# douban/tfmesos

Measured on NVIDIA B200. Metric: ps_push_pull_GBps, higher is better.
Workload: dtype f32

## Files before the change

tfmesos_b200/csrc/psx.cu:

```cuda
#include <cuda.h>
#include <cuda_runtime.h>
#include <unistd.h>

#include <atomic>
#include <cstdarg>
#include <cstdio>
#include <cstring>
#include <mutex>
#include <thread>
#include <unordered_map>
#include <vector>

#include "psx.h"
#include "psx_kernels.cuh"

using namespace psx;

namespace {

thread_local char g_err[512] = "";

int fail(int code, const char *fmt, ...)
{
    va_list ap;
// ... 9 lines not shown
        if (e_ != cudaSuccess)                                                         \
            return fail(PSX_ECUDA, "%s failed: %s (%s:%d)", #expr, cudaGetErrorString(e_), \
                        __FILE__, __LINE__);                                           \
    } while (0)

struct DeviceGuard {
    int prev = -1;
    cudaError_t err = cudaSuccess;
    explicit DeviceGuard(int device)
    {
        err = cudaGetDevice(&prev);
        if (err == cudaSuccess && prev != device) err = cudaSetDevice(device);
        else if (err == cudaSuccess) prev = -1;
    }
    ~DeviceGuard()
    {
        if (prev >= 0) cudaSetDevice(prev);
    }
};
#define PSX_DEVICE(dev)                                                                  \
    DeviceGuard guard_(dev);                                                             \
    if (guard_.err != cudaSuccess)                                                       \
        return fail(PSX_ECUDA, "selecting device %d: %s", (int)(dev), cudaGetErrorString(guard_.err))

typedef CUresult (*WaitValue32Fn)(CUstream, CUdeviceptr, cuuint32_t, unsigned int);
WaitValue32Fn g_wait32 = nullptr;
std::once_flag g_wait_once;

int resolve_memops()
{
    std::call_once(g_wait_once, [] {
        void *fn = nullptr;
        cudaDriverEntryPointQueryResult q;
        if (cudaGetDriverEntryPoint("cuStreamWaitValue32", &fn, cudaEnableDefault, &q) ==
                cudaSuccess &&
            q == cudaDriverEntryPointSuccess)
            g_wait32 = (WaitValue32Fn)fn;
    });
    if (!g_wait32) return fail(PSX_ECUDA, "cuStreamWaitValue32 not available from the driver");
    return PSX_OK;
}

int stream_wait_geq(void *stream, unsigned int *flag, uint32_t value)
{
    int rc = resolve_memops();
    if (rc) return rc;
    CUresult r = g_wait32((CUstream)stream, (CUdeviceptr)(uintptr_t)flag, value,
                          CU_STREAM_WAIT_VALUE_GEQ);
    if (r != CUDA_SUCCESS) return fail(PSX_ECUDA, "cuStreamWaitValue32 failed: CUresult %d", (int)r);
    return PSX_OK;
}

constexpr uint32_t kMagic = 0x50535831u;
constexpr size_t kHeaderBytes = 4096;
constexpr uint64_t kPadElems = 1024;

enum Kind : uint32_t { KIND_SHARD = 1, KIND_CLIENT = 2, KIND_BUFFER = 3, KIND_MAILBOX = 4 };

struct HandleBlob {
    uint32_t magic, abi, kind;
    int32_t device;
    uint64_t pid, local_id, nelem, nelem_pad;
    int32_t opt, n_slots, wire;
    uint32_t pad;
    cudaIpcMemHandle_t ipc;
};
static_assert(sizeof(HandleBlob) == PSX_HANDLE_BYTES, "handle blob size");

int state_arrays(int opt)
{
    switch (opt) {
    case PSX_OPT_SGD: return OptTraits<PSX_OPT_SGD>::kState;
    case PSX_OPT_ADAM: return OptTraits<PSX_OPT_ADAM>::kState;
    case PSX_OPT_MOMENTUM: return OptTraits<PSX_OPT_MOMENTUM>::kState;
    case PSX_OPT_ADAGRAD: return OptTraits<PSX_OPT_ADAGRAD>::kState;
    case PSX_OPT_RMSPROP: return OptTraits<PSX_OPT_RMSPROP>::kState;
    default: return -1;
    }
}

struct Layout {
    uint64_t nelem = 0, nelem_pad = 0;
    int opt = 0, n_slots = 0, wire = 0;
    size_t wire_bytes() const { return wire == PSX_BF16 ? 2 : 4; }
    int n_state() const { return state_arrays(opt); }
    size_t off_var() const { return kHeaderBytes; }
    size_t off_m() const { return off_var() + nelem_pad * 4; }
    size_t off_v() const { return off_m() + (n_state() >= 1 ? nelem_pad * 4 : 0); }
    size_t off_slots() const { return off_v() + (n_state() >= 2 ? nelem_pad * 4 : 0); }
    size_t total() const { return off_slots() + (size_t)n_slots * nelem_pad * wire_bytes(); }
};

struct Mapped {
    char *base = nullptr;
    bool ipc = false;
    int device = 0;
};

struct Bound {
    Mapped grad, param;
    uint64_t elem_off = 0;
    bool valid = false;
};

struct Server;
struct Shard {
    int device = 0;
    Server *server = nullptr;
    std::recursive_mutex serve_mu;
    Layout lay;
    char *base = nullptr;
    int sm_count = 148;
    Mapped client_map[PSX_MAX_SLOTS];
    unsigned int *mirror[PSX_MAX_SLOTS] = {};
    Bound bound[PSX_MAX_SLOTS];
    Mapped mailbox_map[PSX_MAX_SLOTS];
    unsigned int *mailbox[PSX_MAX_SLOTS] = {};
    const float *mc_grad = nullptr;
    float *mc_param = nullptr;
    int mc_members = 0;
    ShardHeader *hdr() const { return (ShardHeader *)base; }
    float *var() const { return (float *)(base + lay.off_var()); }
    float *m() const { return (float *)(base + lay.off_m()); }
    float *v() const { return (float *)(base + lay.off_v()); }
    char *slot(int s) const { return base + lay.off_slots() + (size_t)s * lay.nelem_pad * lay.wire_bytes(); }
};

struct Client {
    int device = 0;
    int slot = 0;
    Layout lay;
    Mapped shard;
    ClientBlock *block = nullptr;
    cudaStream_t poll_stream = nullptr;
    int sm_count = 148;
    ShardHeader *hdr() const { return (ShardHeader *)shard.base; }
    float *var() const { return (float *)(shard.base + lay.off_var()); }
    char *my_slot() const { return shard.base + lay.off_slots() + (size_t)slot * lay.nelem_pad * lay.wire_bytes(); }
};

struct Mailbox {
    int device = 0;
    unsigned int *counter = nullptr;
};

struct TensorList {
    uint64_t client_id = 0;
    int device = 0;
    ListChunk *d_chunks = nullptr;
    int n_chunks = 0;
    int sm_count = 148;
};

struct Buffer {
    int device = 0;
    uint64_t nbytes = 0;
    char *base = nullptr;
};

std::mutex g_mu;
std::unordered_map<uint64_t, Shard *> g_shards;
std::unordered_map<uint64_t, Client *> g_clients;
std::unordered_map<uint64_t, Buffer *> g_buffers;
std::unordered_map<uint64_t, TensorList *> g_lists;
std::unordered_map<uint64_t, Mailbox *> g_mailboxes;
std::atomic<uint64_t> g_next_id{1};
std::atomic<uint64_t> g_launches{0};

template <typename T> T *find(std::unordered_map<uint64_t, T *> &m, uint64_t id)
{
    std::lock_guard<std::mutex> lk(g_mu);
    auto it = m.find(id);
    return it == m.end() ? nullptr : it->second;
}

int sm_count_of(int device)
{
    int n = 148;
    cudaDeviceGetAttribute(&n, cudaDevAttrMultiProcessorCount, device);
    return n > 0 ? n : 148;
}

int enable_peer(int device, int peer);

int open_blob(const HandleBlob &b, int device, Mapped *out)
{
    out->device = b.device;
    if (b.pid == (uint64_t)getpid()) {
        int prc = enable_peer(device, b.device);
        if (prc) return prc;
        std::lock_guard<std::mutex> lk(g_mu);
        char *base = nullptr;
        if (b.kind == KIND_SHARD) {
            auto it = g_shards.find(b.local_id);
            if (it != g_shards.end()) base = it->second->base;
        } else if (b.kind == KIND_CLIENT) {
            auto it = g_clients.find(b.local_id);
            if (it != g_clients.end()) base = (char *)it->second->block;
        } else if (b.kind == KIND_BUFFER) {
            auto it = g_buffers.find(b.local_id);
            if (it != g_buffers.end()) base = it->second->base;
        } else if (b.kind == KIND_MAILBOX) {
            auto it = g_mailboxes.find(b.local_id);
            if (it != g_mailboxes.end()) base = (char *)it->second->counter;
        }
        if (!base) return fail(PSX_EINVAL, "handle refers to an object this process no longer has");
        out->base = base;
        out->ipc = false;
        return PSX_OK;
    }
    PSX_DEVICE(device);
    void *p = nullptr;
    CU_TRY(cudaIpcOpenMemHandle(&p, b.ipc, cudaIpcMemLazyEnablePeerAccess));
    out->base = (char *)p;
    out->ipc = true;
    return PSX_OK;
}

void close_mapped(Mapped &m)
{
    if (m.ipc && m.base) cudaIpcCloseMemHandle(m.base);
    m.base = nullptr;
    m.ipc = false;
}

int check_blob(const void *handle, uint32_t kind, HandleBlob *out)
{
    if (!handle) return fail(PSX_EINVAL, "null handle");
    memcpy(out, handle, sizeof(HandleBlob));
    if (out->magic != kMagic) return fail(PSX_EINVAL, "not a psx handle");
    if (out->abi != PSX_ABI_VERSION)
        return fail(PSX_EABI, "handle from ABI %u, library is ABI %d", out->abi, PSX_ABI_VERSION);
    if (out->kind != kind) return fail(PSX_EINVAL, "handle kind %u, expected %u", out->kind, kind);
    return PSX_OK;
}

int enable_peer(int device, int peer)
{
    if (device == peer) return PSX_OK;
    int can = 0;
    CU_TRY(cudaDeviceCanAccessPeer(&can, device, peer));
    if (!can) return fail(PSX_ECUDA, "device %d cannot access peer %d", device, peer);
    PSX_DEVICE(device);
    cudaError_t e = cudaDeviceEnablePeerAccess(peer, 0);
    if (e == cudaErrorPeerAccessAlreadyEnabled) {
        cudaGetLastError();
        return PSX_OK;
    }
    if (e != cudaSuccess) return fail(PSX_ECUDA, "cudaDeviceEnablePeerAccess(%d->%d): %s", device, peer, cudaGetErrorString(e));
    return PSX_OK;
}

inline int grid_for(size_t work_items, int threads, int sm_count, int ctas_per_sm)
{
    size_t need = (work_items + threads - 1) / threads;
    size_t cap = (size_t)sm_count * ctas_per_sm;
    if (need < 1) need = 1;
    return (int)(need < cap ? need : cap);
}

#define LAUNCH_CHECK()                                                              \
    do {                                                                            \
        cudaError_t e_ = cudaGetLastError();                                        \
        if (e_ != cudaSuccess)                                                      \
            return fail(PSX_ECUDA, "kernel launch failed: %s (%s:%d)",              \
                        cudaGetErrorString(e_), __FILE__, __LINE__);                \
        g_launches.fetch_add(1, std::memory_order_relaxed);                         \
    } while (0)

int launch_copy(void *dst, int dst_t, const void *src, int src_t, uint64_t n, int sm_count,
                unsigned int *ticket, unsigned int *flag, uint32_t seq, cudaStream_t st,
                unsigned int *arrivals = nullptr, unsigned int *stamp_word = nullptr,
                uint32_t stamp = 0)
{
    if (n == 0 && flag == nullptr) return PSX_OK;
    const size_t sb = src_t == PSX_BF16 ? 2 : 4, db = dst_t == PSX_BF16 ? 2 : 4;
    const int vec_ok = (((uintptr_t)src % (4 * sb)) == 0) && (((uintptr_t)dst % (4 * db)) == 0);
    const size_t items = vec_ok ? ((n >> 2) + kCopyUnroll - 1) / kCopyUnroll : n;
    const int grid = grid_for(items ? items : 1, kCopyThreads, sm_count, 8);
#define PSX_COPY(S, D)                                                                        \
    k_copy<S, D><<<grid, kCopyThreads, 0, st>>>((D *)dst, (const S *)src, (size_t)n, vec_ok, \
                                                 ticket, flag, arrivals, seq, stamp_word, stamp)
    if (src_t == PSX_F32 && dst_t == PSX_F32) PSX_COPY(float, float);
    else if (src_t == PSX_F32 && dst_t == PSX_BF16) PSX_COPY(float, __nv_bfloat16);
    else if (src_t == PSX_BF16 && dst_t == PSX_F32) PSX_COPY(__nv_bfloat16, float);
    else if (src_t == PSX_BF16 && dst_t == PSX_BF16) PSX_COPY(__nv_bfloat16, __nv_bfloat16);
    else return fail(PSX_EINVAL, "unknown dtype %d/%d", src_t, dst_t);
#undef PSX_COPY
    LAUNCH_CHECK();
    return PSX_OK;
}

struct ApplyRange {
    size_t off, n;
    int finish;
    unsigned int consume = 0;
    int divisor = 0;
};

template <int OPT, int MODE, bool SCATTER, typename SRC>
void launch_apply_t(Shard *s, SRC src, int count, const PeerSet &peers, cudaStream_t st,
                    const ApplyRange &r)
{
    const size_t n4 = r.n / 4;
    const int grid = grid_for(n4 ? n4 : 1, kApplyThreads, s->sm_count, 3);
    k_apply<OPT, MODE, SCATTER, SRC><<<grid, kApplyThreads, 0, st>>>(
        s->hdr(), (float4 *)(s->var() + r.off), (float4 *)(s->m() + r.off),
        (float4 *)(s->v() + r.off), src, count, n4, peers, r.finish, r.consume,
        r.divisor ? r.divisor : count);
}

template <bool SCATTER, typename SRC>
int launch_apply(Shard *s, int mode, SRC src, int count, const PeerSet &peers, cudaStream_t st,
                 ApplyRange r = ApplyRange{0, 0, 1, 0, 0})
{
    if (r.n == 0 && r.off == 0) r.n = s->lay.nelem_pad;
#define PSX_AP(O, M) launch_apply_t<O, M, SCATTER, SRC>(s, src, count, peers, st, r)
#define PSX_AP3(O)                                                                            \
    if (mode == PSX_MODE_ASYNC_ORDERED) PSX_AP(O, PSX_MODE_ASYNC_ORDERED);                    \
    else if (mode == PSX_MODE_SUM) PSX_AP(O, PSX_MODE_SUM);                                   \
    else if (mode == PSX_MODE_SYNC_MEAN) PSX_AP(O, PSX_MODE_SYNC_MEAN);                       \
    else return fail(PSX_EINVAL, "unknown optimizer/mode %d/%d", opt, mode)
    const int opt = s->lay.opt;
    if (opt == PSX_OPT_SGD) { PSX_AP3(PSX_OPT_SGD); }
    else if (opt == PSX_OPT_ADAM) { PSX_AP3(PSX_OPT_ADAM); }
    else if (opt == PSX_OPT_MOMENTUM) { PSX_AP3(PSX_OPT_MOMENTUM); }
    else if (opt == PSX_OPT_ADAGRAD) { PSX_AP3(PSX_OPT_ADAGRAD); }
    else if (opt == PSX_OPT_RMSPROP) { PSX_AP3(PSX_OPT_RMSPROP); }
    else return fail(PSX_EINVAL, "unknown optimizer/mode %d/%d", opt, mode);
#undef PSX_AP3
#undef PSX_AP
    LAUNCH_CHECK();
    return PSX_OK;
}

struct Shard;
int launch_round_mc(Shard *s, int mode, const PeerSet &peers, cudaStream_t st, const ApplyRange &r);

void fill_mirrors(Shard *s, PeerSet *p)
{
    p->n_mirror = 0;
    p->n_param = 0;
    p->n_mailbox = 0;
    for (int c = 0; c < PSX_MAX_SLOTS; ++c) {
        if (s->mirror[c]) p->mirror[p->n_mirror++] = s->mirror[c];
        if (s->mailbox[c]) p->mailbox[p->n_mailbox++] = s->mailbox[c];
    }
}

int launch_round_mc(Shard *s, int mode, const PeerSet &peers, cudaStream_t st, const ApplyRange &r)
{
    const size_t n4 = r.n / 4;
    const size_t tile = (size_t)kMcThreads * PSX_MC_UNROLL;
    const size_t tiles = (n4 + tile - 1) / tile;
    const size_t cap = (size_t)s->sm_count * PSX_APPLY_MIN_CTAS;
    const int grid = (int)(tiles < 1 ? 1 : (tiles < cap ? tiles : cap));
#define PSX_MC(O, M)                                                                          \
    k_round_mc<O, M, PSX_MC_UNROLL><<<grid, kMcThreads, 0, st>>>(                             \
        s->hdr(), (float4 *)(s->var() + r.off), (float4 *)(s->m() + r.off),                   \
        (float4 *)(s->v() + r.off), s->mc_grad + r.off, s->mc_param + r.off, n4, peers,       \
        r.consume, r.divisor)
    const int opt = s->lay.opt;
#define PSX_MC2(O)                                                                            \
    if (mode == PSX_MODE_SUM) PSX_MC(O, PSX_MODE_SUM);                                        \
    else if (mode == PSX_MODE_SYNC_MEAN) PSX_MC(O, PSX_MODE_SYNC_MEAN);                       \
    else return fail(PSX_EINVAL, "the NVLS round supports SUM / SYNC_MEAN (optimizer/mode %d/%d)", opt, mode)
    if (opt == PSX_OPT_SGD) { PSX_MC2(PSX_OPT_SGD); }
    else if (opt == PSX_OPT_ADAM) { PSX_MC2(PSX_OPT_ADAM); }
    else if (opt == PSX_OPT_MOMENTUM) { PSX_MC2(PSX_OPT_MOMENTUM); }
    else if (opt == PSX_OPT_ADAGRAD) { PSX_MC2(PSX_OPT_ADAGRAD); }
    else if (opt == PSX_OPT_RMSPROP) { PSX_MC2(PSX_OPT_RMSPROP); }
    else return fail(PSX_EINVAL, "the NVLS round supports SUM / SYNC_MEAN (optimizer/mode %d/%d)", opt, mode);
#undef PSX_MC2
#undef PSX_MC
    LAUNCH_CHECK();
    return PSX_OK;
}

struct Server {
    std::thread th;
    std::atomic<bool> stop{false};
    cudaStream_t stream = nullptr;
    int mode = PSX_MODE_ASYNC_ORDERED, aggregate = 1, idle_sleep_us = 0;
    std::atomic<uint64_t> iterations{0};
    std::atomic<int> error{0};
    char errmsg[256] = "";
};

int serve_iteration(Shard *s, Server *sv)
{
    const int n_slots = s->lay.n_slots;
    if (sv->mode == PSX_MODE_ASYNC_ORDERED)
        k_pick<PSX_MODE_ASYNC_ORDERED><<<1, 32, 0, sv->stream>>>(s->hdr(), n_slots, 1);
    else
        k_pick<PSX_MODE_SYNC_MEAN><<<1, 32, 0, sv->stream>>>(s->hdr(), n_slots, sv->aggregate);
    LAUNCH_CHECK();
    PeerSet peers;
    memset(&peers, 0, sizeof(peers));
    const ApplyRange r{0, (size_t)s->lay.nelem_pad, 1, 0, 0};
    if (s->lay.wire == PSX_F32) {
        PickSrc<float> src{(const float *)s->slot(0), (size_t)s->lay.nelem_pad, nullptr};
        return launch_apply<false>(s, sv->mode, src, 0, peers, sv->stream, r);
    }
    PickSrc<__nv_bfloat16> src{(const __nv_bfloat16 *)s->slot(0), (size_t)s->lay.nelem_pad, nullptr};
    return launch_apply<false>(s, sv->mode, src, 0, peers, sv->stream, r);
}

void serve_main(Shard *s, Server *sv)
{
    cudaSetDevice(s->device);
    unsigned int *seen = nullptr;
    cudaError_t e = cudaHostAlloc((void **)&seen, sizeof(unsigned int), cudaHostAllocDefault);
    uint64_t it = 0;
    int idle = 0;
    while (e == cudaSuccess && !sv->stop.load()) {
        e = cudaMemcpyAsync(seen, &s->hdr()->arrivals, sizeof(unsigned int), cudaMemcpyDeviceToHost,
                            sv->stream);
        if (e == cudaSuccess) e = cudaStreamSynchronize(sv->stream);
        if (e != cudaSuccess) break;
        if ((int)*seen < 1) {
            if (sv->idle_sleep_us > 0 && ++idle > 64) usleep((useconds_t)sv->idle_sleep_us);
            continue;
        }
        idle = 0;
        int rc = serve_iteration(s, sv);
        if (rc) {
            snprintf(sv->errmsg, sizeof(sv->errmsg), "%.250s", g_err);
            sv->error.store(rc);
            break;
        }
        sv->iterations.store(++it);
    }
    cudaError_t e2 = cudaStreamSynchronize(sv->stream);
    if (e == cudaSuccess) e = e2;
    if (e != cudaSuccess && sv->error.load() == 0) {
        snprintf(sv->errmsg, sizeof(sv->errmsg), "serving stream: %s", cudaGetErrorString(e));
        sv->error.store(PSX_ECUDA);
    }
    if (seen) cudaFreeHost(seen);
}

int serve_start_impl(Shard *s, int mode, int aggregate, int idle_sleep_us)
{
    if (s->server) return fail(PSX_ESTATE, "shard is already being served");
    if (s->lay.n_slots < 1) return fail(PSX_ESTATE, "serving needs landing slots (n_slots >= 1)");
    if (mode != PSX_MODE_ASYNC_ORDERED && mode != PSX_MODE_SYNC_MEAN)
        return fail(PSX_EINVAL, "serve mode must be ASYNC_ORDERED or SYNC_MEAN");
    if (mode == PSX_MODE_SYNC_MEAN && (aggregate < 1 || aggregate > s->lay.n_slots))
        return fail(PSX_EINVAL, "replicas_to_aggregate %d outside 1..%d", aggregate, s->lay.n_slots);
    if (idle_sleep_us < 0) idle_sleep_us = 0;
    PSX_DEVICE(s->device);
    Server *sv = new Server();
    sv->mode = mode;
    sv->aggregate = aggregate;
    sv->idle_sleep_us = idle_sleep_us;
    cudaError_t e = cudaStreamCreateWithFlags(&sv->stream, cudaStreamNonBlocking);
    if (e != cudaSuccess) {
        delete sv;
        return fail(PSX_ECUDA, "creating the serving stream: %s", cudaGetErrorString(e));
    }
    s->server = sv;
    sv->th = std::thread(serve_main, s, sv);
    return PSX_OK;
}

int serve_stop_impl(Shard *s, int *mode, int *aggregate, int *idle_sleep_us)
{
    Server *sv = s->server;
    if (!sv) return PSX_OK;
    sv->stop.store(true);
    sv->th.join();
    {
        DeviceGuard g(s->device);
        cudaStreamDestroy(sv->stream);
    }
    if (mode) *mode = sv->mode;
    if (aggregate) *aggregate = sv->aggregate;
    if (idle_sleep_us) *idle_sleep_us = sv->idle_sleep_us;
    int err = sv->error.load();
    char msg[256];
    snprintf(msg, sizeof(msg), "%s", sv->errmsg);
    s->server = nullptr;
    delete sv;
    if (err) return fail(err, "serving loop failed: %s", msg);
    return PSX_OK;
}

struct ServePause {
    Shard *s;
    std::unique_lock<std::recursive_mutex> lk;
    bool was = false;
    int mode = 0, aggregate = 1, depth = 0, rc = PSX_OK;
    explicit ServePause(Shard *sh) : s(sh), lk(sh->serve_mu)
    {
        if (s->server) {
            was = true;
            rc = serve_stop_impl(s, &mode, &aggregate, &depth);
        }
    }
    ~ServePause()
    {
        if (was && rc == PSX_OK) serve_start_impl(s, mode, aggregate, depth);
    }
};
#define PSX_PAUSE(shard)              \
    ServePause pause_(shard);         \
    if (pause_.rc) return pause_.rc

int wait_slots(Shard *s, int first, int count, uint32_t wait_seq, void *stream)
{
    if (wait_seq == 0) return PSX_OK;
    for (int k = 0; k < count; ++k) {
        int rc = stream_wait_geq(stream, &s->hdr()->slot_seq[first + k], wait_seq);
        if (rc) return rc;
    }
    return PSX_OK;
}

int check_range(int first, int count, int n_slots)
{
    if (count < 1 || first < 0 || first + count > n_slots || count > PSX_MAX_SLOTS)
        return fail(PSX_EINVAL, "slot range [%d, %d) outside the shard's %d slots", first,
                    first + count, n_slots);
    return PSX_OK;
}

}

extern "C" {

int psx_abi_version(void) { return PSX_ABI_VERSION; }

const char *psx_last_error(void) { return g_err; }

uint64_t psx_launch_count(void) { return g_launches.load(); }

int psx_device_count(int *out_n)
{
    int n = 0;
    cudaError_t e = cudaGetDeviceCount(&n);
    if (out_n) *out_n = (e == cudaSuccess) ? n : 0;
    if (e != cudaSuccess) {
        cudaGetLastError();
        return fail(PSX_ECUDA, "cudaGetDeviceCount: %s", cudaGetErrorString(e));
    }
    if (n == 0) return fail(PSX_ECUDA, "no CUDA device visible");
    return PSX_OK;
}

int psx_init(int device)
{
    int n = 0;
    int rc = psx_device_count(&n);
    if (rc) return rc;
    if (device < 0 || device >= n) return fail(PSX_EINVAL, "device %d out of range [0,%d)", device, n);
    CU_TRY(cudaSetDevice(device));
    CU_TRY(cudaFree(0));
    return resolve_memops();
}

int psx_enable_peer(int device, int peer) { return enable_peer(device, peer); }

int psx_shard_create(int device, uint64_t nelem, int opt, const float *hyper, int n_slots,
                     int wire_dtype, uint64_t *out_id)
{
    if (!out_id || !hyper) return fail(PSX_EINVAL, "null argument");
    if (nelem == 0) return fail(PSX_EINVAL, "empty shard");
    if (state_arrays(opt) < 0) return fail(PSX_EINVAL, "unknown optimizer %d", opt);
    if (opt == PSX_OPT_ADAGRAD && !(hyper[1] > 0.0f))
        return fail(PSX_EINVAL, "Adagrad initial_accumulator_value must be > 0 (got %g)", (double)hyper[1]);
    if (n_slots < 0 || n_slots > PSX_MAX_SLOTS) return fail(PSX_EINVAL, "n_slots %d not in [0,%d]", n_slots, PSX_MAX_SLOTS);
    if (wire_dtype != PSX_F32 && wire_dtype != PSX_BF16) return fail(PSX_EINVAL, "unknown wire dtype %d", wire_dtype);
    PSX_DEVICE(device);
    Shard *s = new Shard();
    s->device = device;
    s->lay.nelem = nelem;
    s->lay.nelem_pad = (nelem + kPadElems - 1) / kPadElems * kPadElems;
    s->lay.opt = opt;
    s->lay.n_slots = n_slots;
    s->lay.wire = wire_dtype;
    s->sm_count = sm_count_of(device);
    void *p = nullptr;
    cudaError_t e = cudaMalloc(&p, s->lay.total());
    if (e != cudaSuccess) {
        size_t total = s->lay.total();
        delete s;
        cudaGetLastError();
        return fail(e == cudaErrorMemoryAllocation ? PSX_ENOMEM : PSX_ECUDA,
                    "cudaMalloc(%zu bytes) for shard: %s", total, cudaGetErrorString(e));
    }
    s->base = (char *)p;
    e = cudaMemset(p, 0, s->lay.total());
    ShardHeader h;
    memset(&h, 0, sizeof(h));
    h.magic = kMagic;
    h.abi = PSX_ABI_VERSION;
    h.lr = hyper[0];
    h.b1 = hyper[1];
    h.b2 = hyper[2];
    h.eps = hyper[3];
    h.b1p = hyper[1];
    h.b2p = hyper[2];
    if (e == cudaSuccess) e = cudaMemcpy(p, &h, sizeof(h), cudaMemcpyHostToDevice);
    const float m0 = opt == PSX_OPT_ADAGRAD ? hyper[1] : opt == PSX_OPT_RMSPROP ? 1.0f : 0.0f;
    if (e == cudaSuccess && m0 != 0.0f) {
        const size_t n4 = s->lay.nelem_pad / 4;
        k_fill<<<grid_for(n4, kCopyThreads, s->sm_count, 8), kCopyThreads>>>((float4 *)s->m(), m0, n4);
        e = cudaGetLastError();
        if (e == cudaSuccess) e = cudaDeviceSynchronize();
        if (e == cudaSuccess) g_launches.fetch_add(1, std::memory_order_relaxed);
    }
    if (e != cudaSuccess) {
        cudaFree(p);
        delete s;
        return fail(PSX_ECUDA, "initialising shard: %s", cudaGetErrorString(e));
    }
    uint64_t id = g_next_id.fetch_add(1);
    {
        std::lock_guard<std::mutex> lk(g_mu);
        g_shards[id] = s;
    }
    *out_id = id;
    return PSX_OK;
}

int psx_shard_destroy(uint64_t id)
{
    Shard *s = nullptr;
    {
        std::lock_guard<std::mutex> lk(g_mu);
        auto it = g_shards.find(id);
        if (it == g_shards.end()) return fail(PSX_EINVAL, "unknown shard id %llu", (unsigned long long)id);
        s = it->second;
        g_shards.erase(it);
    }
    int src;
    {
        std::lock_guard<std::recursive_mutex> lk(s->serve_mu);
        src = serve_stop_impl(s, nullptr, nullptr, nullptr);
    }
    cudaError_t e = cudaSetDevice(s->device);
    if (e == cudaSuccess) e = cudaDeviceSynchronize();
    for (int c = 0; c < PSX_MAX_SLOTS; ++c) {
        close_mapped(s->client_map[c]);
        close_mapped(s->mailbox_map[c]);
        close_mapped(s->bound[c].grad);
        close_mapped(s->bound[c].param);
    }
    cudaError_t e2 = cudaFree(s->base);
    delete s;
    if (e == cudaSuccess) e = e2;
    if (e != cudaSuccess) {
        cudaGetLastError();
        return fail(PSX_ECUDA, "destroying shard %llu: %s", (unsigned long long)id, cudaGetErrorString(e));
    }
    return src;
}

// ... 1048 lines not shown
```

tfmesos_b200/csrc/psx_kernels.cuh:

```cuda
#pragma once

#include <cuda_bf16.h>
#include <cuda_runtime.h>
#include <stddef.h>
#include <stdint.h>

#include "psx.h"

namespace psx {

struct ShardHeader {
    uint32_t magic;
    uint32_t abi;
    float lr, b1, b2, eps;
    float b1p, b2p;
    long long step;
    unsigned int ticket;
    unsigned int apply_seq;
    unsigned int slot_seq[PSX_MAX_SLOTS];
    unsigned int arrivals;
    unsigned int reserved0;
    unsigned int pick_n;
    unsigned int pick[PSX_MAX_SLOTS];
    unsigned int pick_seq[PSX_MAX_SLOTS];
// ... 263 lines not shown
            asm volatile("cp.async.bulk.wait_group.read 1;" ::: "memory");
            issue_one();
            const int s = consumed % kListStages;
            mbar_wait(&full[s], (uint32_t)((consumed / kListStages) & 1));
            asm volatile("fence.proxy.async.shared::cta;" ::: "memory");
            char *dst = to_shard ? shard_base + c.shard_off : c.tensor;
            tma_store_1d(dst, ring + (size_t)s * kListChunkBytes, c.bytes);
            asm volatile("cp.async.bulk.commit_group;" ::: "memory");
            ++consumed;
        }
        asm volatile("cp.async.bulk.wait_group 0;" ::: "memory");
        asm volatile("fence.proxy.async;" ::: "memory");
    }
    for (int j = 0; j < mine; ++j) {
        const ListChunk c = chunk_of(j);
        if (!c.plain) continue;
        const float *src = (const float *)(to_shard ? c.tensor : shard_base + c.shard_off);
        float *dst = (float *)(to_shard ? shard_base + c.shard_off : c.tensor);
        for (uint32_t i = threadIdx.x; i < c.bytes / 4; i += blockDim.x) dst[i] = src[i];
    }
    if (flag != nullptr) {
        if (last_cta(ticket) && threadIdx.x == 0) {
            *ticket = 0;
            __threadfence_system();
            publish_store(flag, seq);
            if (arrivals != nullptr) publish_add(arrivals, 1u);
        }
    }
}

__global__ void __launch_bounds__(kListThreads)
k_list_ldst(const ListChunk *__restrict__ chunks, int n_chunks, char *shard_base, int to_shard,
            unsigned int *ticket, unsigned int *flag, unsigned int *arrivals, unsigned int seq)
{
    for (int j = blockIdx.x; j < n_chunks; j += gridDim.x) {
        const ListChunk c = chunks[j];
        const char *src = to_shard ? c.tensor : shard_base + c.shard_off;
        char *dst = to_shard ? shard_base + c.shard_off : c.tensor;
        if (c.plain) {
            for (uint32_t i = threadIdx.x; i < c.bytes / 4; i += blockDim.x)
                ((float *)dst)[i] = ((const float *)src)[i];
        } else {
            const uint32_t n16 = c.bytes / 16;
            for (uint32_t i = threadIdx.x; i < n16; i += 4 * blockDim.x) {
                float4 r[4];
#pragma unroll
                for (int u = 0; u < 4; ++u)
                    if (i + u * blockDim.x < n16) r[u] = ld_stream((const float4 *)src + i + u * blockDim.x);
#pragma unroll
                for (int u = 0; u < 4; ++u)
                    if (i + u * blockDim.x < n16) st_stream((float4 *)dst + i + u * blockDim.x, r[u]);
            }
        }
    }
    if (flag != nullptr) {
        if (last_cta(ticket) && threadIdx.x == 0) {
            *ticket = 0;
            __threadfence_system();
            publish_store(flag, seq);
            if (arrivals != nullptr) publish_add(arrivals, 1u);
        }
    }
}

__global__ void __launch_bounds__(kCopyThreads) k_fill(float4 *__restrict__ dst, float value, size_t n4)
{
    const float4 v = make_float4(value, value, value, value);
    for (size_t i = (size_t)blockIdx.x * blockDim.x + threadIdx.x; i < n4; i += (size_t)gridDim.x * blockDim.x)
        dst[i] = v;
}

__global__ void k_consume(unsigned int *counter, unsigned int n) { atomicSub(counter, n); }

constexpr int kMaxSignal = 64;
struct SignalSet {
    unsigned int *flag[kMaxSignal];
    unsigned int *arrivals[kMaxSignal];
    int n;
    unsigned int *mailbox;
    unsigned int consume;
};
__global__ void k_signal(SignalSet set, unsigned int seq)
{
    if (set.mailbox != nullptr && threadIdx.x == 0) atomicSub(set.mailbox, set.consume);
    if ((int)threadIdx.x < set.n) {
        __threadfence_system();
        publish_store(set.flag[threadIdx.x], seq);
        publish_add(set.arrivals[threadIdx.x], 1u);
    }
}

template <int OPT> struct OptTraits;
template <> struct OptTraits<PSX_OPT_SGD> { static constexpr int kState = 0; static constexpr bool kPowers = false; };
template <> struct OptTraits<PSX_OPT_ADAM> { static constexpr int kState = 2; static constexpr bool kPowers = true; };
template <> struct OptTraits<PSX_OPT_MOMENTUM> { static constexpr int kState = 1; static constexpr bool kPowers = false; };
template <> struct OptTraits<PSX_OPT_ADAGRAD> { static constexpr int kState = 1; static constexpr bool kPowers = false; };
template <> struct OptTraits<PSX_OPT_RMSPROP> { static constexpr int kState = 2; static constexpr bool kPowers = false; };

__device__ __forceinline__ float sgd1(float var, float g, float lr)
{
    return __fsub_rn(var, __fmul_rn(g, lr));
}

__device__ __forceinline__ void adam1(float &var, float &m, float &v, float g, float alpha,
                                      float omb1, float omb2, float eps)
{
    m = __fadd_rn(m, __fmul_rn(__fsub_rn(g, m), omb1));
    v = __fadd_rn(v, __fmul_rn(__fsub_rn(__fmul_rn(g, g), v), omb2));
    float num = __fmul_rn(m, alpha);
    float den = __fadd_rn(__fsqrt_rn(v), eps);
    var = __fsub_rn(var, __fdiv_rn(num, den));
}

__device__ __forceinline__ void momentum1(float &var, float &a, float g, float lr, float mu)
{
    a = __fadd_rn(__fmul_rn(a, mu), g);
    var = __fsub_rn(var, __fmul_rn(a, lr));
}

__device__ __forceinline__ void adagrad1(float &var, float &a, float g, float lr)
{
    a = __fadd_rn(a, __fmul_rn(g, g));
    var = __fsub_rn(var, __fmul_rn(__fmul_rn(g, lr), __fdiv_rn(1.0f, __fsqrt_rn(a))));
}

__device__ __forceinline__ void rmsprop1(float &var, float &ms, float &mom, float g, float lr,
                                         float omdecay, float mu, float eps)
{
    ms = __fadd_rn(ms, __fmul_rn(__fsub_rn(__fmul_rn(g, g), ms), omdecay));
    mom = __fadd_rn(__fmul_rn(mom, mu), __fdiv_rn(__fmul_rn(g, lr), __fsqrt_rn(__fadd_rn(ms, eps))));
    var = __fsub_rn(var, mom);
}

__device__ __forceinline__ float adam_alpha(float lr, float b1p, float b2p)
{
    float s = __fsqrt_rn(__fsub_rn(1.0f, b2p));
    return __fdiv_rn(__fmul_rn(lr, s), __fsub_rn(1.0f, b1p));
}

template <int OPT>
__device__ __forceinline__ void apply1(float &x, float &m, float &v, float g, float lr, float alpha,
                                       float b1, float b2, float omb1, float omb2, float eps)
{
    if (OPT == PSX_OPT_SGD) x = sgd1(x, g, lr);
    else if (OPT == PSX_OPT_ADAM) adam1(x, m, v, g, alpha, omb1, omb2, eps);
    else if (OPT == PSX_OPT_MOMENTUM) momentum1(x, m, g, lr, b1);
    else if (OPT == PSX_OPT_ADAGRAD) adagrad1(x, m, g, lr);
    else rmsprop1(x, m, v, g, lr, omb1, b2, eps);
}

template <int OPT>
__device__ __forceinline__ void apply4(float4 &x, float4 &m, float4 &v, const float4 &g, float lr,
                                       float alpha, float b1, float b2, float omb1, float omb2,
                                       float eps)
{
    apply1<OPT>(x.x, m.x, v.x, g.x, lr, alpha, b1, b2, omb1, omb2, eps);
    apply1<OPT>(x.y, m.y, v.y, g.y, lr, alpha, b1, b2, omb1, omb2, eps);
    apply1<OPT>(x.z, m.z, v.z, g.z, lr, alpha, b1, b2, omb1, omb2, eps);
    apply1<OPT>(x.w, m.w, v.w, g.w, lr, alpha, b1, b2, omb1, omb2, eps);
}

__device__ __forceinline__ float4 add4(const float4 &a, const float4 &b)
{
    return make_float4(__fadd_rn(a.x, b.x), __fadd_rn(a.y, b.y), __fadd_rn(a.z, b.z),
                       __fadd_rn(a.w, b.w));
}
__device__ __forceinline__ float4 div4(const float4 &a, float d)
{
    return make_float4(__fdiv_rn(a.x, d), __fdiv_rn(a.y, d), __fdiv_rn(a.z, d), __fdiv_rn(a.w, d));
}

template <int OPT, bool SYS_FENCE>
__device__ __forceinline__ void finish_apply(ShardHeader *h, const PeerSet &peers, int applies,
                                             int finish, float b1, float b2)
{
    const bool last = last_cta<SYS_FENCE>(&h->ticket);
    if (last && threadIdx.x == 0 && !finish) {
        h->ticket = 0;
    } else if (last && threadIdx.x == 0) {
        if (OptTraits<OPT>::kPowers) {
            float p1 = h->b1p, p2 = h->b2p;
            for (int k = 0; k < applies; ++k) {
                p1 = __fmul_rn(p1, b1);
                p2 = __fmul_rn(p2, b2);
            }
            h->b1p = p1;
            h->b2p = p2;
        }
        h->step += applies;
        h->ticket = 0;
        const unsigned int seq = h->apply_seq + 1;
        __threadfence_system();
        publish_store(&h->apply_seq, seq);
        for (int c = 0; c < peers.n_mirror; ++c) publish_store(peers.mirror[c], seq);
        for (int c = 0; c < peers.n_mailbox; ++c) publish_add(peers.mailbox[c], 1u);
    }
}

template <int MODE>
__global__ void k_pick(ShardHeader *h, int n_slots, int aggregate)
{
    __shared__ unsigned int s_new[PSX_MAX_SLOTS];
    const int s = threadIdx.x;
    unsigned int seq = 0;
    bool fresh = false;
    if (s < n_slots) {
        seq = ld_sys(&h->slot_seq[s]);
        fresh = seq != h->slot_seen[s];
    }
    if (s < PSX_MAX_SLOTS) s_new[s] = fresh ? seq : 0u;
    __syncthreads();
    if (threadIdx.x != 0) return;
    unsigned int n_new = 0, n_pick = 0;
    if (MODE == PSX_MODE_ASYNC_ORDERED) {
        for (int k = 0; k < n_slots; ++k) {
            if (s_new[k] == 0u) continue;
            h->slot_seen[k] = s_new[k];
            h->pick[n_pick] = (unsigned int)k;
            h->pick_seq[n_pick] = s_new[k];
            ++n_pick;
            ++n_new;
        }
    } else {
        const unsigned int step = (unsigned int)h->step;
        for (int k = 0; k < n_slots; ++k) {
            if (s_new[k] != 0u) {
                h->slot_seen[k] = s_new[k];
                h->pending[k] = 1u;
                h->arrival_rank[k] = ++h->arrival_ctr;
                ++n_new;
            }
            if (h->pending[k] && (int)(ld_sys(&h->slot_stamp[k]) - step) < 0) {
                h->pending[k] = 0u;
                ++h->dropped;
            }
        }
        unsigned int n_pending = 0;
        for (int k = 0; k < n_slots; ++k) n_pending += h->pending[k];
        if (n_pending >= (unsigned int)aggregate) {
            for (int r = 0; r < aggregate; ++r) {
                int best = -1;
                for (int k = 0; k < n_slots; ++k)
                    if (h->pending[k] && (best < 0 || (int)(h->arrival_rank[k] - h->arrival_rank[best]) < 0))
                        best = k;
                h->pending[best] = 0u;
                h->pick[n_pick] = (unsigned int)best;
                h->pick_seq[n_pick] = h->slot_seen[best];
                ++n_pick;
            }
        }
    }
    h->pick_n = n_pick;
    if (n_new) atomicSub(&h->arrivals, n_new);
}

template <int OPT, int MODE>
__device__ __forceinline__ void finish_served(ShardHeader *h, int count, float b1, float b2)
{
    const bool last = last_cta<false>(&h->ticket);
    if (!last || threadIdx.x != 0) return;
    h->ticket = 0;
    if (count == 0) return;
    const int applies = (MODE == PSX_MODE_ASYNC_ORDERED) ? count : 1;
    if (OptTraits<OPT>::kPowers) {
        float p1 = h->b1p, p2 = h->b2p;
        for (int k = 0; k < applies; ++k) {
            p1 = __fmul_rn(p1, b1);
            p2 = __fmul_rn(p2, b2);
        }
        h->b1p = p1;
        h->b2p = p2;
    }
    const long long step0 = h->step;
    h->step = step0 + applies;
    h->served += (unsigned int)count;
    const unsigned int seq = h->apply_seq + 1;
    if (MODE == PSX_MODE_ASYNC_ORDERED) {
        for (int k = 0; k < count; ++k) {
            ClientBlock *cb = (ClientBlock *)h->client_block[h->pick[k]];
            if (cb) cb->step = step0 + k + 1;
        }
    } else {
        for (int c = 0; c < PSX_MAX_SLOTS; ++c) {
            ClientBlock *cb = (ClientBlock *)h->client_block[c];
            if (cb) cb->step = step0 + 1;
        }
    }
    __threadfence_system();
    publish_store(&h->apply_seq, seq);
    if (MODE == PSX_MODE_ASYNC_ORDERED) {
        for (int k = 0; k < count; ++k) {
            ClientBlock *cb = (ClientBlock *)h->client_block[h->pick[k]];
            if (cb) publish_store(&cb->applied, h->pick_seq[k]);
        }
    } else {
        for (int c = 0; c < PSX_MAX_SLOTS; ++c) {
            ClientBlock *cb = (ClientBlock *)h->client_block[c];
            if (cb) publish_add(&cb->tokens, 1u);
        }
    }
}

constexpr int kApplyThreads = 256;
constexpr int kSlotChunk = 4;
#ifndef PSX_APPLY_MIN_CTAS
#define PSX_APPLY_MIN_CTAS 3
#endif
#ifndef PSX_PREFETCH_STATE
#define PSX_PREFETCH_STATE 0
#endif

template <typename WIRE> struct SlotSrc {
    static constexpr bool kPrefetch = false;
    const WIRE *base;
    size_t stride;
    int first;
    __device__ __forceinline__ float4 load(int s, size_t i) const
    {
        return Vec4<WIRE>::load(base + (size_t)(first + s) * stride + 4 * i);
    }
};
template <typename WIRE> struct PeerSrc {
    static constexpr bool kPrefetch = true;
    using wire_t = WIRE;
    PeerSet peers;
    int first;
    __device__ __forceinline__ float4 load(int s, size_t i) const
    {
        return Vec4<WIRE>::load((const WIRE *)peers.grad[first + s] + 4 * i);
    }
};
__device__ __forceinline__ float4 mc_ld_reduce(const float *mc)
{
    float4 v;
    asm volatile("multimem.ld_reduce.relaxed.sys.global.add.v4.f32 {%0,%1,%2,%3}, [%4];"
                 : "=f"(v.x), "=f"(v.y), "=f"(v.z), "=f"(v.w)
                 : "l"(mc)
                 : "memory");
    return v;
}
__device__ __forceinline__ void mc_st(float *mc, const float4 &v)
{
    asm volatile("multimem.st.relaxed.sys.global.v4.f32 [%0], {%1,%2,%3,%4};" ::"l"(mc), "f"(v.x),
                 "f"(v.y), "f"(v.z), "f"(v.w)
                 : "memory");
}
template <typename WIRE> struct PickSrc {
    static constexpr bool kPrefetch = false;
    static constexpr bool kDynamic = true;
    const WIRE *base;
    size_t stride;
    const unsigned int *pick;
    __device__ __forceinline__ float4 load(int s, size_t i) const
    {
        return Vec4<WIRE>::load(base + (size_t)pick[s] * stride + 4 * i);
    }
};
template <typename SRC> struct IsDynamic { static constexpr bool value = false; };
template <typename W> struct IsDynamic<PickSrc<W>> { static constexpr bool value = true; };
template <typename SRC> struct WireOf { using type = float; };
template <typename W> struct WireOf<PeerSrc<W>> { using type = W; };
template <typename SRC> struct IsMulticast { static constexpr bool value = false; };

template <int OPT, int MODE, bool SCATTER, typename SRC>
__global__ void __launch_bounds__(kApplyThreads, PSX_APPLY_MIN_CTAS)
k_apply(ShardHeader *__restrict__ h, float4 *__restrict__ var, float4 *__restrict__ mom,
        float4 *__restrict__ vel, SRC src, int count, size_t n4, PeerSet peers, int finish,
        unsigned int consume, int divisor)
{
    __shared__ unsigned int s_pick[PSX_MAX_SLOTS];
    if constexpr (IsDynamic<SRC>::value) {
        count = (int)h->pick_n;
        divisor = count;
        if (count == 0) n4 = 0;
        if (threadIdx.x < PSX_MAX_SLOTS) s_pick[threadIdx.x] = h->pick[threadIdx.x];
        src.pick = s_pick;
        __syncthreads();
    }
    if (consume != 0 && blockIdx.x == 0 && threadIdx.x == 0) atomicSub(&h->arrivals, consume);
    __shared__ float s_alpha[PSX_MAX_SLOTS];
    const float lr = h->lr, b1 = h->b1, b2 = h->b2, eps = h->eps;
    const float omb1 = __fsub_rn(1.0f, b1);
    const float omb2 = __fsub_rn(1.0f, b2);
    if (OptTraits<OPT>::kPowers) {
        if (threadIdx.x == 0) {
            float p1 = h->b1p, p2 = h->b2p;
            const int na = (MODE == PSX_MODE_ASYNC_ORDERED) ? count : 1;
            for (int k = 0; k < na; ++k) {
                s_alpha[k] = adam_alpha(lr, p1, p2);
                p1 = __fmul_rn(p1, b1);
                p2 = __fmul_rn(p2, b2);
            }
        }
        __syncthreads();
    }
    const float fcount = (float)divisor;

    const size_t stride = (size_t)gridDim.x * blockDim.x;
    size_t i = (size_t)blockIdx.x * blockDim.x + threadIdx.x;
    constexpr bool PF = SRC::kPrefetch;
    float4 gn[kSlotChunk];
    if (PF && i < n4) {
#pragma unroll
        for (int k = 0; k < kSlotChunk; ++k)
            if (k < count) gn[k] = src.load(k, i);
    }
#if PSX_PREFETCH_STATE
    float4 xn = make_float4(0.f, 0.f, 0.f, 0.f), mn = xn, vn = xn;
    if (i < n4) {
        xn = ld_stream(var + i);
        if (OptTraits<OPT>::kState >= 1) mn = ld_stream(mom + i);
        if (OptTraits<OPT>::kState >= 2) vn = ld_stream(vel + i);
    }
#endif
    for (; i < n4; i += stride) {
#if PSX_PREFETCH_STATE
        float4 x = xn, m = mn, v = vn;
        if (i + stride < n4) {
            xn = ld_stream(var + i + stride);
            if (OptTraits<OPT>::kState >= 1) mn = ld_stream(mom + i + stride);
            if (OptTraits<OPT>::kState >= 2) vn = ld_stream(vel + i + stride);
        }
#else
        float4 x = ld_stream(var + i);
        float4 m = make_float4(0.f, 0.f, 0.f, 0.f), v = m;
        if (OptTraits<OPT>::kState >= 1) m = ld_stream(mom + i);
        if (OptTraits<OPT>::kState >= 2) v = ld_stream(vel + i);
#endif
        float4 g[kSlotChunk];
        if (PF) {
#pragma unroll
            for (int k = 0; k < kSlotChunk; ++k) g[k] = gn[k];
            const size_t inext = i + stride;
            if (inext < n4) {
#pragma unroll
                for (int k = 0; k < kSlotChunk; ++k)
                    if (k < count) gn[k] = src.load(k, inext);
            }
        } else {
#pragma unroll
            for (int k = 0; k < kSlotChunk; ++k)
                if (k < count) g[k] = src.load(k, i);
        }
        float4 acc;
        for (int s0 = 0; s0 < count; s0 += kSlotChunk) {
            if (s0 > 0) {
#pragma unroll
                for (int k = 0; k < kSlotChunk; ++k)
                    if (s0 + k < count) g[k] = src.load(s0 + k, i);
            }
            if (MODE == PSX_MODE_ASYNC_ORDERED) {
#pragma unroll
                for (int k = 0; k < kSlotChunk; ++k)
                    if (s0 + k < count)
                        apply4<OPT>(x, m, v, g[k], lr, OptTraits<OPT>::kPowers ? s_alpha[s0 + k] : 0.f,
                                    b1, b2, omb1, omb2, eps);
            } else {
#pragma unroll
                for (int k = 0; k < kSlotChunk; ++k)
                    if (s0 + k < count) acc = (s0 + k == 0) ? g[k] : add4(acc, g[k]);
            }
        }
        if (MODE != PSX_MODE_ASYNC_ORDERED) {
            if (MODE == PSX_MODE_SYNC_MEAN) acc = div4(acc, fcount);
            apply4<OPT>(x, m, v, acc, lr, OptTraits<OPT>::kPowers ? s_alpha[0] : 0.f, b1, b2, omb1,
                        omb2, eps);
        }
        st_stream(var + i, x);
        if (OptTraits<OPT>::kState >= 1) st_stream(mom + i, m);
        if (OptTraits<OPT>::kState >= 2) st_stream(vel + i, v);
        if (SCATTER) {
            using W = typename WireOf<SRC>::type;
            for (int s = 0; s < peers.n_param; ++s)
                Vec4<W>::store((W *)peers.param[s] + 4 * i, x);
        }
    }

    if (IsDynamic<SRC>::value)
        finish_served<OPT, MODE>(h, count, b1, b2);
    else
        finish_apply<OPT, IsMulticast<SRC>::value>(h, peers, (MODE == PSX_MODE_ASYNC_ORDERED) ? count : 1,
                                                    finish, b1, b2);
}

constexpr int kMcThreads = 256;
#ifndef PSX_MC_UNROLL
#define PSX_MC_UNROLL 2
#endif

template <int OPT, int MODE, int U>
__global__ void __launch_bounds__(kMcThreads, PSX_APPLY_MIN_CTAS)
k_round_mc(ShardHeader *__restrict__ h, float4 *__restrict__ var, float4 *__restrict__ mom,
           float4 *__restrict__ vel, const float *grad_mc, float *param_mc, size_t n4,
           PeerSet peers, unsigned int consume, int divisor)
{
    if (consume != 0 && blockIdx.x == 0 && threadIdx.x == 0) atomicSub(&h->arrivals, consume);
    const float lr = h->lr, b1 = h->b1, b2 = h->b2, eps = h->eps;
    const float omb1 = __fsub_rn(1.0f, b1);
    const float omb2 = __fsub_rn(1.0f, b2);
    const float alpha = OptTraits<OPT>::kPowers ? adam_alpha(lr, h->b1p, h->b2p) : 0.f;
    const float fdiv = (float)divisor;

    const size_t tile = (size_t)kMcThreads * U;
    const size_t tiles = (n4 + tile - 1) / tile;
    size_t t = blockIdx.x;
    float4 gn[U];
    if (t < tiles) {
#pragma unroll
        for (int u = 0; u < U; ++u) {
            const size_t i = t * tile + (size_t)u * kMcThreads + threadIdx.x;
            if (i < n4) gn[u] = mc_ld_reduce(grad_mc + 4 * i);
        }
    }
    for (; t < tiles; t += gridDim.x) {
        float4 g[U], x[U], m[U], v[U];
        const size_t base = t * tile + threadIdx.x;
#pragma unroll
        for (int u = 0; u < U; ++u) {
            const size_t i = base + (size_t)u * kMcThreads;
            if (i < n4) {
                x[u] = ld_stream(var + i);
                if (OptTraits<OPT>::kState >= 1) m[u] = ld_stream(mom + i);
                if (OptTraits<OPT>::kState >= 2) v[u] = ld_stream(vel + i);
            }
        }
#pragma unroll
        for (int u = 0; u < U; ++u) g[u] = gn[u];
        const size_t tn = t + gridDim.x;
        if (tn < tiles) {
#pragma unroll
            for (int u = 0; u < U; ++u) {
                const size_t i = tn * tile + (size_t)u * kMcThreads + threadIdx.x;
                if (i < n4) gn[u] = mc_ld_reduce(grad_mc + 4 * i);
            }
        }
#pragma unroll
        for (int u = 0; u < U; ++u) {
            const size_t i = base + (size_t)u * kMcThreads;
            if (i < n4) {
                float4 acc = g[u];
                if (MODE == PSX_MODE_SYNC_MEAN) acc = div4(acc, fdiv);
                apply4<OPT>(x[u], m[u], v[u], acc, lr, alpha, b1, b2, omb1, omb2, eps);
                st_stream(var + i, x[u]);
                if (OptTraits<OPT>::kState >= 1) st_stream(mom + i, m[u]);
                if (OptTraits<OPT>::kState >= 2) st_stream(vel + i, v[u]);
                mc_st(param_mc + 4 * i, x[u]);
            }
        }
    }
    finish_apply<OPT, true>(h, peers, 1, 1, b1, b2);
}

struct RowsHeader {
    unsigned long long count;
    unsigned long long row_len;
};
__host__ __device__ inline size_t rows_idx_off() { return 16; }
__host__ __device__ inline size_t rows_data_off(size_t k) { return (16 + k * 8 + 15) / 16 * 16; }

template <typename SRC, typename DST>
__global__ void __launch_bounds__(kCopyThreads)
k_push_rows(char *slot, const long long *__restrict__ idx, const SRC *__restrict__ rows, size_t k,
            size_t d, unsigned int *ticket, unsigned int *flag, unsigned int *arrivals,
            unsigned int seq)
{
    long long *didx = (long long *)(slot + rows_idx_off());
    DST *drows = (DST *)(slot + rows_data_off(k));
    const size_t tid = (size_t)blockIdx.x * blockDim.x + threadIdx.x;
    const size_t nth = (size_t)gridDim.x * blockDim.x;
    for (size_t i = tid; i < k; i += nth) didx[i] = idx[i];
    for (size_t i = tid; i < k * d; i += nth) drows[i] = from_f32<DST>(to_f32<SRC>(rows[i]));
    if (tid == 0) {
        RowsHeader *rh = (RowsHeader *)slot;
        rh->count = k;
        rh->row_len = d;
    }
    if (last_cta(ticket) && threadIdx.x == 0) {
        *ticket = 0;
        __threadfence_system();
        publish_store(flag, seq);
        publish_add_release(arrivals, 1u);
    }
}

__device__ __forceinline__ long long rows_find(const long long *idx, long long n, long long key)
{
    long long lo = 0, hi = n;
    while (lo < hi) {
        long long mid = (lo + hi) >> 1;
        if (idx[mid] < key) lo = mid + 1;
        else hi = mid;
    }
    return (lo < n && idx[lo] == key) ? lo : -1;
}

template <int OPT, int MODE, typename WIRE>
__global__ void __launch_bounds__(256)
k_apply_rows(ShardHeader *__restrict__ h, float *__restrict__ var, float *__restrict__ mom,
             float *__restrict__ vel, const char *slots, size_t slot_stride, int first, int count,
             size_t d, size_t n_rows, PeerSet peers)
{
    const float lr = h->lr, b1 = h->b1, b2 = h->b2, eps = h->eps;
    const float omb1 = __fsub_rn(1.0f, b1), omb2 = __fsub_rn(1.0f, b2);
    const float alpha = OptTraits<OPT>::kPowers ? adam_alpha(lr, h->b1p, h->b2p) : 0.f;
    const float fcount = (float)count;
    const int lane = threadIdx.x & 31;
    const size_t warp = ((size_t)blockIdx.x * blockDim.x + threadIdx.x) >> 5;
    const size_t n_warps = ((size_t)gridDim.x * blockDim.x) >> 5;
    size_t total = 0;
    for (int s = 0; s < count; ++s)
        total += ((const RowsHeader *)(slots + (size_t)(first + s) * slot_stride))->count;
    for (size_t e = warp; e < total; e += n_warps) {
        int w = 0;
        size_t k = e;
        for (;; ++w) {
            const size_t c = ((const RowsHeader *)(slots + (size_t)(first + w) * slot_stride))->count;
            if (k < c) break;
            k -= c;
        }
        const char *sw = slots + (size_t)(first + w) * slot_stride;
        const size_t kw = ((const RowsHeader *)sw)->count;
        const long long row = ((const long long *)(sw + rows_idx_off()))[k];
        if (row < 0 || (size_t)row >= n_rows) continue;
        bool rep = true;
        for (int w2 = 0; w2 < w && rep; ++w2) {
            const char *s2 = slots + (size_t)(first + w2) * slot_stride;
            if (rows_find((const long long *)(s2 + rows_idx_off()),
                          (long long)((const RowsHeader *)s2)->count, row) >= 0)
                rep = false;
        }
        if (!rep) continue;
        long long pos[PSX_MAX_SLOTS];
        for (int w2 = w + 1; w2 < count; ++w2) {
            const char *s2 = slots + (size_t)(first + w2) * slot_stride;
            pos[w2] = rows_find((const long long *)(s2 + rows_idx_off()),
                                (long long)((const RowsHeader *)s2)->count, row);
        }
        const WIRE *g0 = (const WIRE *)(sw + rows_data_off(kw)) + k * d;
        for (size_t j = lane; j < d; j += 32) {
            float g = to_f32<WIRE>(g0[j]);
            for (int w2 = w + 1; w2 < count; ++w2) {
                if (pos[w2] < 0) continue;
                const char *s2 = slots + (size_t)(first + w2) * slot_stride;
                const size_t k2 = ((const RowsHeader *)s2)->count;
                g = __fadd_rn(g, to_f32<WIRE>(((const WIRE *)(s2 + rows_data_off(k2)))[(size_t)pos[w2] * d + j]));
            }
            if (MODE == PSX_MODE_SYNC_MEAN) g = __fdiv_rn(g, fcount);
            const size_t at = (size_t)row * d + j;
            float x = var[at], m = 0.f, v = 0.f;
            if (OptTraits<OPT>::kState >= 1) m = mom[at];
            if (OptTraits<OPT>::kState >= 2) v = vel[at];
            apply1<OPT>(x, m, v, g, lr, alpha, b1, b2, omb1, omb2, eps);
            if (OptTraits<OPT>::kState >= 1) mom[at] = m;
            if (OptTraits<OPT>::kState >= 2) vel[at] = v;
            var[at] = x;
        }
    }
    finish_apply<OPT, false>(h, peers, 1, 1, b1, b2);
}

}
```

Before: 1529.

## Tile apply kernel with per-optimizer unroll and occupancy-sized grid

Replaces the grid-stride apply loop, which used a one-step gradient prefetch, with a tiled loop. Each thread handles several float4 elements per tile, and the unroll count is derived from how many state arrays the optimizer touches, so roughly eight loads are in flight per thread. The grid is now sized from the tile count and from the occupancy API instead of a fixed three CTAs per SM. This aims to raise memory-level parallelism on the peer-gradient and state streams, at the cost of more registers per thread and the loss of cross-iteration prefetch.

```diff
diff --git a/tfmesos_b200/csrc/psx.cu b/tfmesos_b200/csrc/psx.cu
--- a/tfmesos_b200/csrc/psx.cu
+++ b/tfmesos_b200/csrc/psx.cu
@@ -335,8 +335,18 @@
 void launch_apply_t(Shard *s, SRC src, int count, const PeerSet &peers, cudaStream_t st,
                     const ApplyRange &r)
 {
+    static const int ctas_per_sm = [] {
+        int n = 0;
+        if (cudaOccupancyMaxActiveBlocksPerMultiprocessor(&n, k_apply<OPT, MODE, SCATTER, SRC>,
+                                                          kApplyThreads, 0) != cudaSuccess || n < 1) {
+            cudaGetLastError();
+            n = kApplyMinCtas;
+        }
+        return n;
+    }();
     const size_t n4 = r.n / 4;
-    const int grid = grid_for(n4 ? n4 : 1, kApplyThreads, s->sm_count, 3);
+    const size_t tile = (size_t)kApplyThreads * ApplyTile<OPT>::kU;
+    const int grid = grid_for((n4 + tile - 1) / tile, 1, s->sm_count, ctas_per_sm);
     k_apply<OPT, MODE, SCATTER, SRC><<<grid, kApplyThreads, 0, st>>>(
         s->hdr(), (float4 *)(s->var() + r.off), (float4 *)(s->m() + r.off),
         (float4 *)(s->v() + r.off), src, count, n4, peers, r.finish, r.consume,
@@ -386,7 +396,7 @@
     const size_t n4 = r.n / 4;
     const size_t tile = (size_t)kMcThreads * PSX_MC_UNROLL;
     const size_t tiles = (n4 + tile - 1) / tile;
-    const size_t cap = (size_t)s->sm_count * PSX_APPLY_MIN_CTAS;
+    const size_t cap = (size_t)s->sm_count * kMcMinCtas;
     const int grid = (int)(tiles < 1 ? 1 : (tiles < cap ? tiles : cap));
 #define PSX_MC(O, M)                                                                          \
     k_round_mc<O, M, PSX_MC_UNROLL><<<grid, kMcThreads, 0, st>>>(                             \
diff --git a/tfmesos_b200/csrc/psx_kernels.cuh b/tfmesos_b200/csrc/psx_kernels.cuh
--- a/tfmesos_b200/csrc/psx_kernels.cuh
+++ b/tfmesos_b200/csrc/psx_kernels.cuh
@@ -589,16 +589,16 @@
 }
 
 constexpr int kApplyThreads = 256;
+constexpr int kApplyMinCtas = 3;
+constexpr int kApplyLoads = 8;
 constexpr int kSlotChunk = 4;
-#ifndef PSX_APPLY_MIN_CTAS
-#define PSX_APPLY_MIN_CTAS 3
-#endif
-#ifndef PSX_PREFETCH_STATE
-#define PSX_PREFETCH_STATE 0
-#endif
+template <int OPT> struct ApplyTile {
+    static constexpr int kArrays = 2 + OptTraits<OPT>::kState;
+    static constexpr int kU = (kApplyLoads + kArrays - 1) / kArrays;
+    static constexpr int kSlots = kU >= kSlotChunk ? 1 : kSlotChunk / kU;
+};
 
 template <typename WIRE> struct SlotSrc {
-    static constexpr bool kPrefetch = false;
     const WIRE *base;
     size_t stride;
     int first;
@@ -608,7 +608,6 @@
     }
 };
 template <typename WIRE> struct PeerSrc {
-    static constexpr bool kPrefetch = true;
     using wire_t = WIRE;
     PeerSet peers;
     int first;
@@ -633,7 +632,6 @@
                  : "memory");
 }
 template <typename WIRE> struct PickSrc {
-    static constexpr bool kPrefetch = false;
     static constexpr bool kDynamic = true;
     const WIRE *base;
     size_t stride;
@@ -650,7 +648,7 @@
 template <typename SRC> struct IsMulticast { static constexpr bool value = false; };
 
 template <int OPT, int MODE, bool SCATTER, typename SRC>
-__global__ void __launch_bounds__(kApplyThreads, PSX_APPLY_MIN_CTAS)
+__global__ void __launch_bounds__(kApplyThreads, kApplyMinCtas)
 k_apply(ShardHeader *__restrict__ h, float4 *__restrict__ var, float4 *__restrict__ mom,
         float4 *__restrict__ vel, SRC src, int count, size_t n4, PeerSet peers, int finish,
         unsigned int consume, int divisor)
@@ -683,83 +681,66 @@
     }
     const float fcount = (float)divisor;
 
-    const size_t stride = (size_t)gridDim.x * blockDim.x;
-    size_t i = (size_t)blockIdx.x * blockDim.x + threadIdx.x;
-    constexpr bool PF = SRC::kPrefetch;
-    float4 gn[kSlotChunk];
-    if (PF && i < n4) {
-#pragma unroll
-        for (int k = 0; k < kSlotChunk; ++k)
-            if (k < count) gn[k] = src.load(k, i);
-    }
-#if PSX_PREFETCH_STATE
-    float4 xn = make_float4(0.f, 0.f, 0.f, 0.f), mn = xn, vn = xn;
-    if (i < n4) {
-        xn = ld_stream(var + i);
-        if (OptTraits<OPT>::kState >= 1) mn = ld_stream(mom + i);
-        if (OptTraits<OPT>::kState >= 2) vn = ld_stream(vel + i);
-    }
-#endif
-    for (; i < n4; i += stride) {
-#if PSX_PREFETCH_STATE
-        float4 x = xn, m = mn, v = vn;
-        if (i + stride < n4) {
-            xn = ld_stream(var + i + stride);
-            if (OptTraits<OPT>::kState >= 1) mn = ld_stream(mom + i + stride);
-            if (OptTraits<OPT>::kState >= 2) vn = ld_stream(vel + i + stride);
-        }
-#else
-        float4 x = ld_stream(var + i);
-        float4 m = make_float4(0.f, 0.f, 0.f, 0.f), v = m;
-        if (OptTraits<OPT>::kState >= 1) m = ld_stream(mom + i);
-        if (OptTraits<OPT>::kState >= 2) v = ld_stream(vel + i);
-#endif
-        float4 g[kSlotChunk];
-        if (PF) {
-#pragma unroll
-            for (int k = 0; k < kSlotChunk; ++k) g[k] = gn[k];
-            const size_t inext = i + stride;
-            if (inext < n4) {
-#pragma unroll
-                for (int k = 0; k < kSlotChunk; ++k)
-                    if (k < count) gn[k] = src.load(k, inext);
-            }
-        } else {
-#pragma unroll
-            for (int k = 0; k < kSlotChunk; ++k)
-                if (k < count) g[k] = src.load(k, i);
-        }
-        float4 acc;
-        for (int s0 = 0; s0 < count; s0 += kSlotChunk) {
-            if (s0 > 0) {
-#pragma unroll
-                for (int k = 0; k < kSlotChunk; ++k)
-                    if (s0 + k < count) g[k] = src.load(s0 + k, i);
-            }
-            if (MODE == PSX_MODE_ASYNC_ORDERED) {
-#pragma unroll
-                for (int k = 0; k < kSlotChunk; ++k)
-                    if (s0 + k < count)
-                        apply4<OPT>(x, m, v, g[k], lr, OptTraits<OPT>::kPowers ? s_alpha[s0 + k] : 0.f,
-                                    b1, b2, omb1, omb2, eps);
-            } else {
-#pragma unroll
-                for (int k = 0; k < kSlotChunk; ++k)
-                    if (s0 + k < count) acc = (s0 + k == 0) ? g[k] : add4(acc, g[k]);
-            }
-        }
-        if (MODE != PSX_MODE_ASYNC_ORDERED) {
-            if (MODE == PSX_MODE_SYNC_MEAN) acc = div4(acc, fcount);
-            apply4<OPT>(x, m, v, acc, lr, OptTraits<OPT>::kPowers ? s_alpha[0] : 0.f, b1, b2, omb1,
-                        omb2, eps);
-        }
-        st_stream(var + i, x);
-        if (OptTraits<OPT>::kState >= 1) st_stream(mom + i, m);
-        if (OptTraits<OPT>::kState >= 2) st_stream(vel + i, v);
-        if (SCATTER) {
-            using W = typename WireOf<SRC>::type;
-            for (int s = 0; s < peers.n_param; ++s)
-                Vec4<W>::store((W *)peers.param[s] + 4 * i, x);
+    constexpr int U = ApplyTile<OPT>::kU, KS = ApplyTile<OPT>::kSlots;
+    constexpr size_t tile = (size_t)kApplyThreads * U;
+    const size_t tiles = (n4 + tile - 1) / tile;
+    for (size_t t = blockIdx.x; t < tiles; t += gridDim.x) {
+        const size_t base = t * tile + threadIdx.x;
+        const size_t left = n4 - t * tile;
+        const int live = left < tile ? (int)left : (int)tile;
+        float4 x[U], m[U], v[U], g[KS][U], acc[U];
+#pragma unroll
+        for (int u = 0; u < U; ++u) {
+            const size_t i = base + (size_t)u * kApplyThreads;
+            x[u] = m[u] = v[u] = acc[u] = make_float4(0.f, 0.f, 0.f, 0.f);
+            if ((int)threadIdx.x + u * kApplyThreads < live) {
+                x[u] = ld_stream(var + i);
+                if (OptTraits<OPT>::kState >= 1) m[u] = ld_stream(mom + i);
+                if (OptTraits<OPT>::kState >= 2) v[u] = ld_stream(vel + i);
+            }
+        }
+        for (int s0 = 0; s0 < count; s0 += KS) {
+#pragma unroll
+            for (int k = 0; k < KS; ++k)
+#pragma unroll
+                for (int u = 0; u < U; ++u) {
+                    const size_t i = base + (size_t)u * kApplyThreads;
+                    g[k][u] = make_float4(0.f, 0.f, 0.f, 0.f);
+                    if (s0 + k < count && (int)threadIdx.x + u * kApplyThreads < live)
+                        g[k][u] = src.load(s0 + k, i);
+                }
+#pragma unroll
+            for (int k = 0; k < KS; ++k) {
+                if (s0 + k < count) {
+#pragma unroll
+                    for (int u = 0; u < U; ++u) {
+                        if (MODE == PSX_MODE_ASYNC_ORDERED)
+                            apply4<OPT>(x[u], m[u], v[u], g[k][u], lr,
+                                        OptTraits<OPT>::kPowers ? s_alpha[s0 + k] : 0.f, b1, b2, omb1,
+                                        omb2, eps);
+                        else
+                            acc[u] = (s0 + k == 0) ? g[k][u] : add4(acc[u], g[k][u]);
+                    }
+                }
+            }
+        }
+#pragma unroll
+        for (int u = 0; u < U; ++u) {
+            const size_t i = base + (size_t)u * kApplyThreads;
+            if ((int)threadIdx.x + u * kApplyThreads >= live) continue;
+            if (MODE != PSX_MODE_ASYNC_ORDERED) {
+                if (MODE == PSX_MODE_SYNC_MEAN) acc[u] = div4(acc[u], fcount);
+                apply4<OPT>(x[u], m[u], v[u], acc[u], lr, OptTraits<OPT>::kPowers ? s_alpha[0] : 0.f,
+                            b1, b2, omb1, omb2, eps);
+            }
+            st_stream(var + i, x[u]);
+            if (OptTraits<OPT>::kState >= 1) st_stream(mom + i, m[u]);
+            if (OptTraits<OPT>::kState >= 2) st_stream(vel + i, v[u]);
+            if (SCATTER) {
+                using W = typename WireOf<SRC>::type;
+                for (int s = 0; s < peers.n_param; ++s)
+                    Vec4<W>::store((W *)peers.param[s] + 4 * i, x[u]);
+            }
         }
     }
 
@@ -774,9 +755,10 @@
 #ifndef PSX_MC_UNROLL
 #define PSX_MC_UNROLL 2
 #endif
+constexpr int kMcMinCtas = 3;
 
 template <int OPT, int MODE, int U>
-__global__ void __launch_bounds__(kMcThreads, PSX_APPLY_MIN_CTAS)
+__global__ void __launch_bounds__(kMcThreads, kMcMinCtas)
 k_round_mc(ShardHeader *__restrict__ h, float4 *__restrict__ var, float4 *__restrict__ mom,
            float4 *__restrict__ vel, const float *grad_mc, float *param_mc, size_t n4,
            PeerSet peers, unsigned int consume, int divisor)
```

Result: no change. 1519 (median of 6 runs) (-0.7%).
